# TARTRL/Deepfake_Detection

Measured on NVIDIA H100. Metric: images/sec (device-timed, max over ranks) efficientnet_b0 3x224x224 train step, higher is better.
Workload: dtype bf16

## Files before the change

### deepfake_detection_b200/csrc/dwconv.cu

```cuda
#include <stdlib.h>

#include "common.cuh"
#include "bn_finalize.cuh"

namespace {

constexpr int CB = 64;
constexpr int P = 8;
constexpr int NTHREADS = 256;
constexpr int DW_MAX_SMEM = 200 * 1024;


struct DwGeom {
    int N, H, W, C, Ho, Wo, pad;
    int TH, TW;
    int IH, IW;
    int tiles_x, tiles_y;
    int dbg;
    float* part;
};

__device__ __forceinline__ void load_chan_params(const float* p, int cbase, int C, float* out, float dflt) {
#pragma unroll
    for (int i = 0; i < 8; i++) out[i] = (p && cbase + i < C) ? p[cbase + i] : dflt;
}

constexpr int UNR = 4;
template <typename T, int ACT, bool AFFINE, int CPW = 32>
__device__ __forceinline__ void stage_input_tile(uint32_t* tile, const T* __restrict__ img, int H, int W, int C,
                                                 int c0, int iy0, int ix0, int IH, int IW,
                                                 const float* __restrict__ scale, const float* __restrict__ shift) {
    constexpr int VPP = CPW / 4;
    const int v = threadIdx.x % VPP;
    const int cbase = c0 + v * 8;
    const bool cvalid = cbase < C;
    float sc[8], sh[8];
    if (AFFINE) { load_chan_params(scale, cbase, C, sc, 1.f); load_chan_params(shift, cbase, C, sh, 0.f); }
    const int npix = IH * IW;
    const int PSTEP = blockDim.x / VPP;
    const int dq = PSTEP / IW, dr = PSTEP - dq * IW;
    int r = (threadIdx.x / VPP) / IW, c = (threadIdx.x / VPP) - r * IW;
    for (int base = threadIdx.x / VPP; base < npix; base += PSTEP * UNR) {
        uint4 raw[UNR];
        bool ok[UNR];
#pragma unroll
        for (int u = 0; u < UNR; u++) {
            const int pix = base + u * PSTEP;
// ... 15 lines not shown
#pragma unroll
                    for (int i = 0; i < 8; i++) {
                        float uu = AFFINE ? fmaf(f[i], sc[i], sh[i]) : f[i];
                        f[i] = act_fwd<ACT>(uu);
                    }
                    o = pack8<T>(f);
                } else {
                    o = raw[u];
                }
            }
            *reinterpret_cast<uint4*>(tile + pix * CPW + v * 4) = o;
        }
    }
}

template <typename T, bool AFFINE, int UG_ = 0, int CPW = 32>
__device__ __forceinline__ void stage_grad_tile(uint32_t* tile, const T* __restrict__ g, const T* __restrict__ y,
                                                int Ho, int Wo, int C, int c0, int oy0, int ox0, int IH, int IW,
                                                const float* __restrict__ cA, const float* __restrict__ cB,
                                                const float* __restrict__ cC) {
    constexpr int VPP = CPW / 4;
    const int v = threadIdx.x % VPP;
    const int cbase = c0 + v * 8;
    const bool cvalid = cbase < C;
    float A[8], B[8], Cc[8];
    if (AFFINE) { load_chan_params(cA, cbase, C, A, 1.f); load_chan_params(cB, cbase, C, B, 0.f); load_chan_params(cC, cbase, C, Cc, 0.f); }
    const int npix = IH * IW;
    const int PSTEP = blockDim.x / VPP;
    constexpr int UG = UG_ ? UG_ : (AFFINE ? 2 : 4);
    const int dq = PSTEP / IW, dr = PSTEP - dq * IW;
    int r = (threadIdx.x / VPP) / IW, c = (threadIdx.x / VPP) - r * IW;
    for (int base = threadIdx.x / VPP; base < npix; base += PSTEP * UG) {
        uint4 graw[UG], yraw[UG];
        bool ok[UG];
#pragma unroll
        for (int u = 0; u < UG; u++) {
            const int pix = base + u * PSTEP;
            const int oy = oy0 + r, ox = ox0 + c;
            ok[u] = pix < npix && cvalid && oy >= 0 && oy < Ho && ox >= 0 && ox < Wo;
            if (ok[u]) {
                const uint32_t off = (uint32_t)((oy * Wo + ox) * C + cbase);
                graw[u] = ldg16(g + off);
                if (AFFINE) yraw[u] = ldg16(y + off);
            }
// ... 10 lines not shown
                    float gg[8], yy[8];
                    unpack8<T>(graw[u], gg);
                    unpack8<T>(yraw[u], yy);
#pragma unroll
                    for (int i = 0; i < 8; i++) gg[i] = fmaf(A[i], gg[i], fmaf(B[i], yy[i], Cc[i]));
                    o = pack8<T>(gg);
                } else {
                    o = graw[u];
                }
            }
            *reinterpret_cast<uint4*>(tile + pix * CPW + v * 4) = o;
        }
    }
}

template <typename T, int K>
__device__ __forceinline__ void strip_dgrad_s2(const uint32_t* __restrict__ tile, int IW, int sy, int sx, int lane,
                                               const float (&w)[K * K][2], float (&acc)[P][2]) {
    constexpr int PAD = (K - 1) / 2;
#pragma unroll
    for (int kh = 0; kh < K; kh++) {
        const int q = sy + PAD - kh;
        if (q & 1) continue;
        const int row = (q >> 1) + 1;
        const uint32_t* rp = tile + (row * IW + (sx >> 1)) * 32 + lane;
        float2 vv[P / 2 + 2];
#pragma unroll
        for (int j = 0; j < P / 2 + 2; j++) vv[j] = unpack2<T>(rp[j * 32]);
#pragma unroll
        for (int p = 0; p < P; p++) {
// ... 45 lines not shown
    }
    __syncthreads();
    if (threadIdx.x < 2 * CPW) {
        float s = 0.f;
#pragma unroll
        for (int w = 0; w < (int)(blockDim.x >> 5); w++) s += sm[w * 64 + threadIdx.x];
        fn(threadIdx.x, s);
    }
    __syncthreads();
}

template <typename T, int K, int S, int ACT, bool AFFINE, int NT, int CPW = 32, int DT = 0, int DL = 0>
__global__ void __launch_bounds__(NT)
dwconv_fwd_kernel(const T* __restrict__ x, const float* __restrict__ scale, const float* __restrict__ shift,
                  const float* __restrict__ wgt, T* __restrict__ out, double* __restrict__ dsum,
                  double* __restrict__ dsq, const BnFinDesc* __restrict__ fin, DwGeom g) {
    extern __shared__ __align__(16) uint32_t tile[];
    __shared__ float red[NTHREADS / 32 * 64];
    constexpr int SUB = 32 / CPW;
    const int warp = threadIdx.x >> 5, lane = threadIdx.x & 31;
    const int cp = lane % CPW, sub = lane / CPW;
    const int tx = blockIdx.x % g.tiles_x, ty = blockIdx.x / g.tiles_x;
    const int c0 = blockIdx.y * (2 * CPW), n = blockIdx.z;
    const int oy0 = ty * g.TH, ox0 = tx * g.TW;
    const T* img = x + (size_t)n * g.H * g.W * g.C;
    stage_input_tile<T, ACT, AFFINE, CPW>(tile, img, g.H, g.W, g.C, c0, oy0 * S - (g.pad - DT), ox0 * S - (g.pad - DL), g.IH, g.IW, scale, shift);

    const int ch = c0 + cp * 2;
    const bool chv = ch < g.C;
    float w[K * K][2];
#pragma unroll
    for (int i = 0; i < K * K; i++) {
        w[i][0] = chv ? wgt[(size_t)ch * K * K + i] : 0.f;
        w[i][1] = chv ? wgt[(size_t)(ch + 1) * K * K + i] : 0.f;
    }
    __syncthreads();

    float s0 = 0.f, s1 = 0.f, q0 = 0.f, q1 = 0.f;
    const int strips_x = g.TW / P;
    const int xsh = 31 - __clz(strips_x);
    const int nstrips = ((g.TH + SUB - 1) / SUB) * strips_x;
    T* oimg = out + (size_t)n * g.Ho * g.Wo * g.C;
    for (int s = warp; s < nstrips; s += (int)(blockDim.x >> 5)) {
        const int sy = (s >> xsh) * SUB + sub, sx = (s & (strips_x - 1)) * P;
        int oy = oy0 + sy, ox = ox0 + sx;
        if (sy >= g.TH || oy >= g.Ho || ox >= g.Wo) continue;
        float acc[P][2];
#pragma unroll
        for (int p = 0; p < P; p++) { acc[p][0] = 0.f; acc[p][1] = 0.f; }
        strip_conv<T, K, S, CPW>(tile, g.IW, sy * S, sx * S, cp, w, acc);
        if (chv) {
#pragma unroll
            for (int p = 0; p < P; p++) {
                if (ox + p < g.Wo) {
                    uint32_t pk = pack2<T>(acc[p][0], acc[p][1]);
                    *reinterpret_cast<uint32_t*>(oimg + (uint32_t)((oy * g.Wo + ox + p) * g.C + ch)) = pk;
                    float2 r = unpack2<T>(pk);
                    s0 += r.x; s1 += r.y;
                    q0 = fmaf(r.x, r.x, q0); q1 = fmaf(r.y, r.y, q1);
                }
            }
        }
    }
    if (dsum) {
        double* ps = stat_slot(dsum, g.C);
        double* pq = stat_slot(dsq, g.C);
        reduce_warps_emit<CPW>(red, s0, s1, [&](int c, float v) { if (c0 + c < g.C) atomicAdd(ps + c0 + c, (double)v); });
        reduce_warps_emit<CPW>(red, q0, q1, [&](int c, float v) { if (c0 + c < g.C) atomicAdd(pq + c0 + c, (double)v); });
    }
    bn_finalize_tail(fin, threadIdx.x, NT);
}

template <typename T, int K, int S, int MODE, bool AFFINE, int NT>
__global__ void __launch_bounds__(NT)
dwconv_dgrad_kernel(const T* __restrict__ gy, const T* __restrict__ yout, const float* __restrict__ cA,
                    const float* __restrict__ cB, const float* __restrict__ cC, const float* __restrict__ wgt,
                    const T* __restrict__ xin, const float* __restrict__ scale, const float* __restrict__ shift,
                    const float* __restrict__ mean, const float* __restrict__ rstd, const T* __restrict__ add,
                    T* __restrict__ gx, double* __restrict__ ds1, double* __restrict__ ds2, DwGeom g) {
    extern __shared__ __align__(16) uint32_t tile[];
    __shared__ float red[NTHREADS / 32 * 64];
// ... 217 lines not shown
        }
    }
}

template <typename T, int K, int S, bool AFFINE, int MODE, int NT, int P, int CPW = 32, int DT = 0, int DL = 0>
#ifndef DW_BWD_OCC3
#define DW_BWD_OCC3 4
#endif
__global__ void __launch_bounds__(NT, K == 3 ? (P == 4 ? DW_BWD_OCC3 : 3) : 2)
dwconv_bwd_kernel(const T* __restrict__ gy, const T* __restrict__ yout, const float* __restrict__ cA,
                  const float* __restrict__ cB, const float* __restrict__ cC, const float* __restrict__ wgt,
                  const T* __restrict__ xin, const float* __restrict__ scale, const float* __restrict__ shift,
                  const float* __restrict__ mean, const float* __restrict__ rstd, const T* __restrict__ add,
                  T* __restrict__ gx,
                  float* __restrict__ dW, double* __restrict__ ds1, double* __restrict__ ds2,
                  const BnBwdFinDesc* __restrict__ fin, DwGeom g) {
    extern __shared__ __align__(16) uint32_t tile[];
    __shared__ float red[NTHREADS / 32 * 64];
    const int warp = threadIdx.x >> 5, lane = threadIdx.x & 31;
    constexpr int NW = NT / 32;
    constexpr int SUB = 32 / CPW;
    constexpr int CW = 2 * CPW;
    const int cp = lane % CPW, sub = lane / CPW;
    const int tx = blockIdx.x % g.tiles_x, ty = blockIdx.x / g.tiles_x;
    const int c0 = blockIdx.y * CW;
    const int y0 = ty * g.TH, x0 = tx * g.TW;
    const int pp = K - 1 - g.pad;
    const int ch = c0 + cp * 2;
    const bool chv = ch < g.C;
    float w[K * K][2], wacc[K * K][2];
#pragma unroll
    for (int i = 0; i < K * K; i++) {
        const int src = S == 1 ? (K * K - 1 - i) : i;
// ... 7 lines not shown
        mu0 = mean[ch]; mu1 = mean[ch + 1]; rs0 = rstd[ch]; rs1 = rstd[ch + 1];
    }
    const float nm0 = -mu0 * rs0, nm1 = -mu1 * rs1;
    float a0 = 0.f, a1 = 0.f, b0 = 0.f, b1 = 0.f;
    const int strips_x = g.TW / P;
    const int xsh = 31 - __clz(strips_x);
    const int row_groups = S == 1 ? (g.TH + SUB - 1) / SUB : ((g.TH + 1) / 2 + SUB - 1) / SUB;
    const int nstrips = (S == 1 ? row_groups : 2 * row_groups) * strips_x;
    auto strip_row = [&](int s) {
        const int r = s >> xsh;
        if (S == 1) return r * SUB + sub;
        const int par = r >= row_groups ? 1 : 0;
        return 2 * ((r - par * row_groups) * SUB + sub) + par;
    };

    for (int n = blockIdx.z; n < g.N; n += gridDim.z) {
        const size_t ooff = (size_t)n * g.Ho * g.Wo * g.C;
        const size_t ioff = (size_t)n * g.H * g.W * g.C;
        const T* xin_n = xin + ioff;
        T* gx_n = gx + ioff;
        uint32_t pre[P];
        auto prefetch = [&](int s) {
            const int sy = strip_row(s), sx = (s & (strips_x - 1)) * P;
            const int iy = y0 + sy, ix = x0 + sx;
            const bool rowok = chv && sy < g.TH && iy < g.H;
            const uint32_t off0 = (uint32_t)((iy * g.W + ix) * g.C + ch);
#pragma unroll
            for (int p = 0; p < P; p++)
                pre[p] = (rowok && ix + p < g.W) ? __ldg(reinterpret_cast<const uint32_t*>(xin_n + off0 + (uint32_t)(p * g.C))) : 0u;
        };
        if (warp < nstrips) prefetch(warp);
        __syncthreads();
        if (!(g.dbg & 2))
            stage_grad_tile<T, AFFINE, (K == 5 ? 4 : 2), CPW>(tile, gy + ooff, AFFINE ? yout + ooff : nullptr, g.Ho, g.Wo, g.C, c0,
                                   S == 1 ? y0 - pp : (y0 >> 1) - 1, S == 1 ? x0 - pp : (x0 >> 1) - 1, g.IH, g.IW, cA, cB, cC);
        __syncthreads();
        if (!(g.dbg & 1))
        for (int s = warp; s < nstrips; s += NW) {
            const int sy = strip_row(s), sx = (s & (strips_x - 1)) * P;
            const int iy = y0 + sy, ix = x0 + sx;
            float av[P][2], da[P][2], xh[P][2];
            const bool interior = sy < g.TH && iy < g.H && ix + P <= g.W;
#pragma unroll
            for (int p = 0; p < P; p++) {
                const float2 xi = unpack2<T>(pre[p]);
                if (MODE == 1) {
                    const float u0 = fmaf(xi.x, sc0, sh0), u1 = fmaf(xi.y, sc1, sh1);
                    const float g0 = sigmoid_fast(u0), g1 = sigmoid_fast(u1);
                    const float2 ar = unpack2<T>(pack2<T>(u0 * g0, u1 * g1));
                    av[p][0] = ar.x;
                    av[p][1] = ar.y;
// ... 193 lines not shown
    } while (0)

extern "C" {

static int dw_fwd(const void* x, const float* scale, const float* shift, const float* w, void* out, int N, int H, int W,
                  int C, int k, int stride, int dt_, int dl_, int act_in, int dt, double* dsum, double* dsq,
                  const void* fin, void* stream) {
    if (C % 8 || N <= 0 || H <= 0 || W <= 0) return dfd_set_error(DFD_ERR_ARG, "dfd_dwconv_fwd: sizes");
    const bool relu = act_in == DFD_ACT_RELU;
    if (relu && (k != 3 || stride != 1 || dt_ || dl_ || dsum || dsq || fin))
        return dfd_set_error(DFD_ERR_UNSUPPORTED, "dfd_dwconv_fwd: a ReLU input needs k = 3, stride 1 and no statistics");
    if (!relu && !scale && act_in != DFD_ACT_NONE) return dfd_set_error(DFD_ERR_ARG, "dfd_dwconv_fwd: act without BN");
    if (!relu && scale && act_in != DFD_ACT_SWISH) return dfd_set_error(DFD_ERR_UNSUPPORTED, "dfd_dwconv_fwd: BN input implies Swish");
    DwGeom g;
    const int cpw = dw_cpw(C);
    int smem = fill_geom(g, N, H, W, C, k, stride, false, cpw);
    if (dt_ || dl_) {
        if (stride != 2 || !scale || dw_nt(k) != (k == 5 ? 128 : 256))
            return dfd_set_error(DFD_ERR_UNSUPPORTED, "dfd_dwconv_fwd_pad: asymmetric pads need stride 2, a BN + Swish input and the default CTA size");
        dim3 grid(g.tiles_x * g.tiles_y, (C + 2 * cpw - 1) / (2 * cpw), N);
        cudaStream_t st = (cudaStream_t)stream;
#define FWP1(K_, CPW_, DT_, DL_) do { constexpr int NT = K_ == 5 ? 128 : 256;                                                  \
        DW_LAUNCH((dwconv_fwd_kernel<T, K_, 2, DFD_ACT_SWISH, true, NT, CPW_, DT_, DL_>), grid, smem, st, (const T*)x, scale, shift, w, \
                  (T*)out, dsum, dsq, (const BnFinDesc*)fin, g); } while (0)
#define FWP2(K_, DT_, DL_) do { if (cpw == 32) FWP1(K_, 32, DT_, DL_); else if (cpw == 16) FWP1(K_, 16, DT_, DL_); else FWP1(K_, 8, DT_, DL_); } while (0)
#define FWP(K_) do { if (dt_ && dl_) FWP2(K_, 1, 1); else if (dt_) FWP2(K_, 1, 0); else FWP2(K_, 0, 1); } while (0)
        DW_DISPATCH_T(dt, {
            if (k == 3) FWP(3);
            else if (k == 5) FWP(5);
            else return dfd_set_error(DFD_ERR_UNSUPPORTED, "depthwise conv: k in {3,5}, stride in {1,2}");
        });
#undef FWP
#undef FWP2
#undef FWP1
        DFD_LAUNCH_CHECK();
        return DFD_OK;
    }
    dim3 grid(g.tiles_x * g.tiles_y, (C + 2 * cpw - 1) / (2 * cpw), N);
    cudaStream_t st = (cudaStream_t)stream;
#define FW(ACT_, AFF_, CPW_) DW_LAUNCH((dwconv_fwd_kernel<T, K, S, ACT_, AFF_, NT, CPW_>), grid, smem, st, (const T*)x, scale, shift, w, (T*)out, dsum, dsq, (const BnFinDesc*)fin, g)
#define FWC(ACT_, AFF_) do { if (cpw == 32) FW(ACT_, AFF_, 32); else if (cpw == 16) FW(ACT_, AFF_, 16); else FW(ACT_, AFF_, 8); } while (0)
    if (relu) {
        DW_DISPATCH_T(dt, { constexpr int K = 3, S = 1; DW_NT(3, {
            if (scale) FWC(DFD_ACT_RELU, true);
            else FWC(DFD_ACT_RELU, false);
        }); });
        DFD_LAUNCH_CHECK();
        return DFD_OK;
    }
    DW_DISPATCH_T(dt, DW_DISPATCH_KS(k, stride, {
        if (scale) FWC(DFD_ACT_SWISH, true);
        else FWC(DFD_ACT_NONE, false);
    }));
#undef FWC
#undef FW
// ... 82 lines not shown
    return tiles * gz;
}

static int dw_bwd(const void* gy, const void* yout, const float* cA, const float* cB, const float* cC,
                  const float* w, const void* xin, const float* scale, const float* shift, const float* mean,
                  const float* rstd, const void* add, void* gx, float* dW, int N, int H, int W, int C, int k,
                  int stride, int dt_, int dl_, int dt, double* s1, double* s2, void* ws, long long ws_bytes, const void* fin,
                  void* stream, bool relu = false) {
    if (C % 8 || N <= 0 || H <= 0 || W <= 0) return dfd_set_error(DFD_ERR_ARG, "dfd_dwconv_bwd: sizes");
    if (relu && (k != 3 || stride != 1 || cA || dt_ || dl_))
        return dfd_set_error(DFD_ERR_UNSUPPORTED, "dfd_dwconv_bwd_relu: k = 3, stride 1, the BN backward not folded into gy (cA NULL)");
    if (!xin || !dW) return dfd_set_error(DFD_ERR_ARG, "dfd_dwconv_bwd: operands");
    if (scale && (!shift || !mean || !rstd || !s1 || !s2)) return dfd_set_error(DFD_ERR_ARG, "dfd_dwconv_bwd: mode 1 operands");
    DwGeom g;
    const int cpw = dw_cpw(C);
    int smem = fill_geom(g, N, H, W, C, k, stride, true, cpw);
    constexpr int NT = 128;
    const int red_bytes = (NT / 32) * k * k * 2 * cpw * (int)sizeof(float);
    if (smem < red_bytes) smem = red_bytes;
    int tiles, cbs, gz;
    dw_bwd_grid(g, N, C, cpw, tiles, cbs, gz);
    if (ws) {
        if ((long long)cbs * tiles * gz * k * k * 2 * cpw * 4 > ws_bytes)
            return dfd_set_error(DFD_ERR_ARG, "dfd_dwconv_bwd: workspace too small (blocks x dfd_dwconv_bwd_parts x block_channels*k*k floats)");
        g.part = (float*)ws;
    }
    dim3 grid(tiles, cbs, gz);
    cudaStream_t st = (cudaStream_t)stream;
    static int pb3 = 0, pb5 = 0;
    if (!pb3) { const char* e3 = getenv("DFD_DW_PB3"); const char* e5 = getenv("DFD_DW_PB5"); pb3 = (e3 && atoi(e3) == 8) ? 8 : 4; pb5 = (e5 && atoi(e5) == 4) ? 4 : 8; }
    const int pb = k == 3 ? pb3 : pb5;
#define BWARGS (const T*)gy, (const T*)yout, cA, cB, cC, w, (const T*)xin, scale, shift, mean, rstd, (const T*)add, (T*)gx, dW, s1, s2, (const BnBwdFinDesc*)fin, g
#define BW1(K_, S_, AFF, MODE_) do {                                                                                          \
        constexpr int PD = K_ == 3 ? 4 : 8;                                                                                   \
        if (cpw == 16) DW_LAUNCH((dwconv_bwd_kernel<T, K_, S_, AFF, MODE_, NT, PD, 16>), grid, smem, st, BWARGS);             \
        else if (cpw == 8) DW_LAUNCH((dwconv_bwd_kernel<T, K_, S_, AFF, MODE_, NT, PD, 8>), grid, smem, st, BWARGS);          \
        else if (pb == 4) DW_LAUNCH((dwconv_bwd_kernel<T, K_, S_, AFF, MODE_, NT, 4>), grid, smem, st, BWARGS);               \
        else DW_LAUNCH((dwconv_bwd_kernel<T, K_, S_, AFF, MODE_, NT, 8>), grid, smem, st, BWARGS);                            \
    } while (0)
#define BW(K_, S_) do { if (scale) { if (cA) BW1(K_, S_, true, 1); else BW1(K_, S_, false, 1); } else { if (cA) BW1(K_, S_, true, 0); else BW1(K_, S_, false, 0); } } while (0)
#define BWP1(K_, DT_, DL_) do {                                                                                               \
        constexpr int PD = K_ == 3 ? 4 : 8;                                                                                   \
        if (cpw == 16) DW_LAUNCH((dwconv_bwd_kernel<T, K_, 2, true, 1, NT, PD, 16, DT_, DL_>), grid, smem, st, BWARGS);       \
        else if (cpw == 8) DW_LAUNCH((dwconv_bwd_kernel<T, K_, 2, true, 1, NT, PD, 8, DT_, DL_>), grid, smem, st, BWARGS);    \
        else DW_LAUNCH((dwconv_bwd_kernel<T, K_, 2, true, 1, NT, PD, 32, DT_, DL_>), grid, smem, st, BWARGS);                 \
    } while (0)
#define BWP(K_) do { if (dt_ && dl_) BWP1(K_, 1, 1); else if (dt_) BWP1(K_, 1, 0); else BWP1(K_, 0, 1); } while (0)
// ... 62 lines not shown
```

### deepfake_detection_b200/csrc/gemm_tc.cu

```cuda
#include <cuda.h>
#include <stdio.h>
#include <stdlib.h>

#include <type_traits>

#include "common.cuh"
#include "bn_finalize.cuh"

namespace {

constexpr int BLOCK_M = 128;
constexpr int BLOCK_K = 64;
constexpr int MMA_K = 16;
constexpr int SLAB = 64;
constexpr int NUM_THREADS = 384;
constexpr int EPI_THREADS = 256;
constexpr int MAX_BLOCK_N = 128;
constexpr int SMEM_BUDGET = 224 * 1024;

__device__ __forceinline__ uint32_t smem_addr(const void* p) { return (uint32_t)__cvta_generic_to_shared(p); }

__device__ __forceinline__ void mbar_init(uint64_t* bar, uint32_t count) {
    asm volatile("mbarrier.init.shared::cta.b64 [%0], %1;" ::"r"(smem_addr(bar)), "r"(count));
}
__device__ __forceinline__ void mbar_arrive_expect_tx(uint64_t* bar, uint32_t bytes) {
    asm volatile("mbarrier.arrive.expect_tx.shared::cta.b64 _, [%0], %1;" ::"r"(smem_addr(bar)), "r"(bytes) : "memory");
}
__device__ __forceinline__ void mbar_arrive(uint64_t* bar) {
    asm volatile("mbarrier.arrive.shared::cta.b64 _, [%0];" ::"r"(smem_addr(bar)) : "memory");
}
__device__ __forceinline__ void mbar_wait(uint64_t* bar, uint32_t parity) {
    uint32_t addr = smem_addr(bar);
    asm volatile(
        "{\n"
        ".reg .pred p;\n"
        "WAIT_LOOP:\n"
        "mbarrier.try_wait.parity.shared::cta.b64 p, [%0], %1;\n"
        "@p bra WAIT_DONE;\n"
        "bra WAIT_LOOP;\n"
        "WAIT_DONE:\n"
        "}\n" ::"r"(addr), "r"(parity) : "memory");
}

__device__ __forceinline__ void tma_load_2d(void* smem_dst, const CUtensorMap* map, uint64_t* bar, int c0, int c1) {
    asm volatile(
        "cp.async.bulk.tensor.2d.shared::cluster.global.mbarrier::complete_tx::bytes [%0], [%1, {%3, %4}], [%2];"
        ::"r"(smem_addr(smem_dst)), "l"(reinterpret_cast<uint64_t>(map)), "r"(smem_addr(bar)), "r"(c0), "r"(c1)
        : "memory");
}
__device__ __forceinline__ void tma_store_2d(const CUtensorMap* map, const void* smem_src, int c0, int c1) {
    asm volatile("cp.async.bulk.tensor.2d.global.shared::cta.bulk_group [%0, {%2, %3}], [%1];"
                 ::"l"(reinterpret_cast<uint64_t>(map)), "r"(smem_addr(smem_src)), "r"(c0), "r"(c1) : "memory");
}
__device__ __forceinline__ void tma_load_4d(void* smem_dst, const CUtensorMap* map, uint64_t* bar, int c0, int c1, int c2, int c3) {
    asm volatile(
        "cp.async.bulk.tensor.4d.shared::cluster.global.mbarrier::complete_tx::bytes [%0], [%1, {%3, %4, %5, %6}], [%2];"
        ::"r"(smem_addr(smem_dst)), "l"(reinterpret_cast<uint64_t>(map)), "r"(smem_addr(bar)), "r"(c0), "r"(c1), "r"(c2), "r"(c3)
        : "memory");
}
__device__ __forceinline__ void tma_store_4d(const CUtensorMap* map, const void* smem_src, int c0, int c1, int c2, int c3) {
    asm volatile("cp.async.bulk.tensor.4d.global.shared::cta.bulk_group [%0, {%2, %3, %4, %5}], [%1];"
                 ::"l"(reinterpret_cast<uint64_t>(map)), "r"(smem_addr(smem_src)), "r"(c0), "r"(c1), "r"(c2), "r"(c3) : "memory");
}
__device__ __forceinline__ void tma_reduce_add_4d(const CUtensorMap* map, const void* smem_src, int c0, int c1, int c2, int c3) {
    asm volatile("cp.reduce.async.bulk.tensor.4d.global.shared::cta.add.tile.bulk_group [%0, {%2, %3, %4, %5}], [%1];"
                 ::"l"(reinterpret_cast<uint64_t>(map)), "r"(smem_addr(smem_src)), "r"(c0), "r"(c1), "r"(c2), "r"(c3) : "memory");
}
__device__ __forceinline__ void tma_store_commit() { asm volatile("cp.async.bulk.commit_group;" ::: "memory"); }
template <int N> __device__ __forceinline__ void tma_store_wait_read() {
    asm volatile("cp.async.bulk.wait_group.read %0;" ::"n"(N) : "memory");
}
__device__ __forceinline__ void prefetch_tmap(const CUtensorMap* map) {
    asm volatile("prefetch.tensormap [%0];" ::"l"(reinterpret_cast<uint64_t>(map)) : "memory");
}

__device__ __forceinline__ void wgmma_fence() { asm volatile("wgmma.fence.sync.aligned;" ::: "memory"); }
__device__ __forceinline__ void wgmma_commit() { asm volatile("wgmma.commit_group.sync.aligned;" ::: "memory"); }
template <int N> __device__ __forceinline__ void wgmma_wait() { asm volatile("wgmma.wait_group.sync.aligned %0;" ::"n"(N) : "memory"); }
__device__ __forceinline__ void wgmma_wait_all() { wgmma_wait<0>(); }
template <int R> __device__ __forceinline__ void fence_acc(float (&d)[R]) {
#pragma unroll
    for (int i = 0; i < R; i++) asm volatile("" : "+f"(d[i])::"memory");
}

template <typename T, int TA, int TB>
__device__ __forceinline__ void wgmma_n64(float (&d)[32], uint64_t adesc, uint64_t bdesc, uint32_t accumulate) {
    if constexpr (std::is_same<T, bf16>::value) {
        asm volatile(
            "{\n.reg .pred p;\nsetp.ne.b32 p, %34, 0;\n"
// ... 435 lines not shown
    for (int j = 0; j < BN / 8; j++) {
        const float s0 = odd ? acc[4 * j] : acc[4 * j + 2], s1 = odd ? acc[4 * j + 1] : acc[4 * j + 3];
        const float o0 = __shfl_xor_sync(0xffffffffu, s0, 1), o1 = __shfl_xor_sync(0xffffffffu, s1, 1);
        const float4 v = odd ? make_float4(o0, o1, acc[4 * j + 2], acc[4 * j + 3]) : make_float4(acc[4 * j], acc[4 * j + 1], o0, o1);
        const int col = n0 + 8 * j + cb;
        if (8 * j < p.block_n && row < p.Nw && col < p.Kw) {
            float* dst = base + (size_t)row * p.Kw + col;
            if (p.part) *reinterpret_cast<float4*>(dst) = v;
            else
                asm volatile("red.global.add.v4.f32 [%0], {%1, %2, %3, %4};" ::"l"(dst), "f"(v.x), "f"(v.y), "f"(v.z), "f"(v.w)
                             : "memory");
        }
    }
}

typedef CUresult (*EncodeTiledFn)(CUtensorMap*, CUtensorMapDataType, cuuint32_t, void*, const cuuint64_t*,
                                  const cuuint64_t*, const cuuint32_t*, const cuuint32_t*, CUtensorMapInterleave,
                                  CUtensorMapSwizzle, CUtensorMapL2promotion, CUtensorMapFloatOOBfill);

static EncodeTiledFn get_encode_fn() {
    static EncodeTiledFn fn = nullptr;
    if (!fn) {
        void* p = nullptr;
        cudaDriverEntryPointQueryResult qres;
        if (cudaGetDriverEntryPoint("cuTensorMapEncodeTiled", &p, cudaEnableDefault, &qres) == cudaSuccess &&
            qres == cudaDriverEntryPointSuccess)
            fn = (EncodeTiledFn)p;
    }
    return fn;
}

static int make_map(CUtensorMap* m, const void* base, long long rows, int cols, int box_rows, int is_bf16) {
    EncodeTiledFn fn = get_encode_fn();
    if (!fn) return dfd_set_error(DFD_ERR_CUDA, "cuTensorMapEncodeTiled entry point not available");
    cuuint64_t dims[2] = {(cuuint64_t)cols, (cuuint64_t)rows};
    cuuint64_t strides[1] = {(cuuint64_t)cols * 2};
    cuuint32_t box[2] = {(cuuint32_t)BLOCK_K, (cuuint32_t)box_rows};
    cuuint32_t estr[2] = {1, 1};
    CUresult r = fn(m, is_bf16 ? CU_TENSOR_MAP_DATA_TYPE_BFLOAT16 : CU_TENSOR_MAP_DATA_TYPE_FLOAT16, 2,
                    const_cast<void*>(base), dims, strides, box, estr, CU_TENSOR_MAP_INTERLEAVE_NONE,
                    CU_TENSOR_MAP_SWIZZLE_128B, CU_TENSOR_MAP_L2_PROMOTION_L2_256B, CU_TENSOR_MAP_FLOAT_OOB_FILL_NONE);
    if (r != CUDA_SUCCESS) {
        char buf[160];
        snprintf(buf, sizeof(buf), "cuTensorMapEncodeTiled failed (%d) rows=%lld cols=%d box_rows=%d", (int)r, rows, cols, box_rows);
        return dfd_set_error(DFD_ERR_CUDA, buf);
    }
    return DFD_OK;
}


struct PixelView { long long sW, sH, sN; };
static int make_map_nhwc(CUtensorMap* m, const void* base, int N, int H, int W, int C, int bw, int bh, int bn, int is_bf16,
                         int es = 1, const PixelView* pv = nullptr) {
    EncodeTiledFn fn = get_encode_fn();
    if (!fn) return dfd_set_error(DFD_ERR_CUDA, "cuTensorMapEncodeTiled entry point not available");
    cuuint64_t dims[4] = {(cuuint64_t)C, (cuuint64_t)W, (cuuint64_t)H, (cuuint64_t)N};
    cuuint64_t strides[3] = {(cuuint64_t)C * 2, (cuuint64_t)W * C * 2, (cuuint64_t)H * W * C * 2};
    if (pv) { strides[0] = (cuuint64_t)pv->sW; strides[1] = (cuuint64_t)pv->sH; strides[2] = (cuuint64_t)pv->sN; }
    cuuint32_t box[4] = {(cuuint32_t)BLOCK_K, (cuuint32_t)((bw - 1) * es + 1), (cuuint32_t)((bh - 1) * es + 1), (cuuint32_t)bn};
    cuuint32_t estr[4] = {1, (cuuint32_t)es, (cuuint32_t)es, 1};
    CUresult r = fn(m, is_bf16 ? CU_TENSOR_MAP_DATA_TYPE_BFLOAT16 : CU_TENSOR_MAP_DATA_TYPE_FLOAT16, 4,
                    const_cast<void*>(base), dims, strides, box, estr, CU_TENSOR_MAP_INTERLEAVE_NONE,
                    CU_TENSOR_MAP_SWIZZLE_128B, CU_TENSOR_MAP_L2_PROMOTION_L2_256B, CU_TENSOR_MAP_FLOAT_OOB_FILL_NONE);
    if (r != CUDA_SUCCESS) {
        char buf[200];
        snprintf(buf, sizeof(buf), "cuTensorMapEncodeTiled (4-D) failed (%d) N=%d H=%d W=%d C=%d box=%dx%dx%d", (int)r, N, H, W, C, bw, bh, bn);
        return dfd_set_error(DFD_ERR_CUDA, buf);
    }
    return DFD_OK;
}

template <typename T, int BN>
static void launch_tc_kernel(int grid, size_t smem, cudaStream_t st, const CUtensorMap& ma, const CUtensorMap& mb,
                             const CUtensorMap& mc, const TcParams& p) {
    static bool attr = false;
    if (!attr) { cudaFuncSetAttribute(gemm_tc_kernel<T, BN>, cudaFuncAttributeMaxDynamicSharedMemorySize, SMEM_BUDGET); attr = true; }
    gemm_tc_kernel<T, BN><<<grid, NUM_THREADS, smem, st>>>(ma, mb, mc, p);
}

template <typename T, int BN>
static void launch_wgrad_kernel(dim3 grid, size_t smem, cudaStream_t st, const CUtensorMap& mg, const CUtensorMap& mx, float* dW,
                                const WgParams& p) {
    static bool attr = false;
    if (!attr) { cudaFuncSetAttribute(wgrad_tc_kernel<T, BN>, cudaFuncAttributeMaxDynamicSharedMemorySize, 100 * 1024); attr = true; }
    wgrad_tc_kernel<T, BN><<<grid, WG_THREADS, smem, st>>>(mg, mx, dW, p);
// ... 315 lines not shown
```

Before: 11470.

## Stage depthwise conv input and gradient tiles via TMA with double-buffered prefetch

```diff
diff --git a/deepfake_detection_b200/csrc/dwconv.cu b/deepfake_detection_b200/csrc/dwconv.cu
--- a/deepfake_detection_b200/csrc/dwconv.cu
+++ b/deepfake_detection_b200/csrc/dwconv.cu
@@ -2,6 +2,7 @@
 
 #include "common.cuh"
 #include "bn_finalize.cuh"
+#include "tma.cuh"
 
 namespace {
 
@@ -26,11 +27,11 @@
 }
 
 constexpr int UNR = 4;
-template <typename T, int ACT, bool AFFINE, int CPW = 32>
+template <typename T, int ACT, bool AFFINE>
 __device__ __forceinline__ void stage_input_tile(uint32_t* tile, const T* __restrict__ img, int H, int W, int C,
                                                  int c0, int iy0, int ix0, int IH, int IW,
                                                  const float* __restrict__ scale, const float* __restrict__ shift) {
-    constexpr int VPP = CPW / 4;
+    constexpr int CPW = 32, VPP = CPW / 4;
     const int v = threadIdx.x % VPP;
     const int cbase = c0 + v * 8;
     const bool cvalid = cbase < C;
@@ -76,12 +77,12 @@
     }
 }
 
-template <typename T, bool AFFINE, int UG_ = 0, int CPW = 32>
+template <typename T, bool AFFINE>
 __device__ __forceinline__ void stage_grad_tile(uint32_t* tile, const T* __restrict__ g, const T* __restrict__ y,
                                                 int Ho, int Wo, int C, int c0, int oy0, int ox0, int IH, int IW,
                                                 const float* __restrict__ cA, const float* __restrict__ cB,
                                                 const float* __restrict__ cC) {
-    constexpr int VPP = CPW / 4;
+    constexpr int CPW = 32, VPP = CPW / 4;
     const int v = threadIdx.x % VPP;
     const int cbase = c0 + v * 8;
     const bool cvalid = cbase < C;
@@ -89,7 +90,7 @@
     if (AFFINE) { load_chan_params(cA, cbase, C, A, 1.f); load_chan_params(cB, cbase, C, B, 0.f); load_chan_params(cC, cbase, C, Cc, 0.f); }
     const int npix = IH * IW;
     const int PSTEP = blockDim.x / VPP;
-    constexpr int UG = UG_ ? UG_ : (AFFINE ? 2 : 4);
+    constexpr int UG = AFFINE ? 2 : 4;
     const int dq = PSTEP / IW, dr = PSTEP - dq * IW;
     int r = (threadIdx.x / VPP) / IW, c = (threadIdx.x / VPP) - r * IW;
     for (int base = threadIdx.x / VPP; base < npix; base += PSTEP * UG) {
@@ -130,6 +131,76 @@
     }
 }
 
+template <typename T, int ACT, bool AFFINE, int CPW>
+__device__ __forceinline__ void activate_tile(uint32_t* __restrict__ tile, int H, int W, int C, int c0, int iy0, int ix0,
+                                              int IH, int IW, const float* __restrict__ scale, const float* __restrict__ shift) {
+    constexpr int VPP = CPW / 4;
+    const int v = threadIdx.x % VPP;
+    const int cbase = c0 + v * 8;
+    const bool cvalid = cbase < C;
+    float sc[8], sh[8];
+    if (AFFINE) { load_chan_params(scale, cbase, C, sc, 1.f); load_chan_params(shift, cbase, C, sh, 0.f); }
+    const int npix = IH * IW;
+    const int PSTEP = blockDim.x / VPP;
+    const int dq = PSTEP / IW, dr = PSTEP - dq * IW;
+    int r = (threadIdx.x / VPP) / IW, c = (threadIdx.x / VPP) - r * IW;
+#pragma unroll 4
+    for (int pix = threadIdx.x / VPP; pix < npix; pix += PSTEP) {
+        const int iy = iy0 + r, ix = ix0 + c;
+        const bool ok = cvalid && iy >= 0 && iy < H && ix >= 0 && ix < W;
+        uint4* q = reinterpret_cast<uint4*>(tile + pix * CPW + v * 4);
+        uint4 o = make_uint4(0, 0, 0, 0);
+        if (ok) {
+            float f[8];
+            unpack8<T>(*q, f);
+#pragma unroll
+            for (int i = 0; i < 8; i++) f[i] = act_fwd<ACT>(AFFINE ? fmaf(f[i], sc[i], sh[i]) : f[i]);
+            o = pack8<T>(f);
+        }
+        *q = o;
+        r += dq; c += dr;
+        if (c >= IW) { c -= IW; r++; }
+    }
+}
+
+template <typename T, bool AFFINE, int CPW>
+__device__ __forceinline__ void form_grad_tile(uint32_t* __restrict__ dyt, const uint32_t* __restrict__ rg,
+                                               const uint32_t* __restrict__ ry, int Ho, int Wo, int C, int c0, int oy0,
+                                               int ox0, int IH, int IW, const float* __restrict__ cA,
+                                               const float* __restrict__ cB, const float* __restrict__ cC) {
+    constexpr int VPP = CPW / 4;
+    const int v = threadIdx.x % VPP;
+    const int cbase = c0 + v * 8;
+    const bool cvalid = cbase < C;
+    float A[8], B[8], Cc[8];
+    if (AFFINE) { load_chan_params(cA, cbase, C, A, 1.f); load_chan_params(cB, cbase, C, B, 0.f); load_chan_params(cC, cbase, C, Cc, 0.f); }
+    const int npix = IH * IW;
+    const int PSTEP = blockDim.x / VPP;
+    const int dq = PSTEP / IW, dr = PSTEP - dq * IW;
+    int r = (threadIdx.x / VPP) / IW, c = (threadIdx.x / VPP) - r * IW;
+#pragma unroll 4
+    for (int pix = threadIdx.x / VPP; pix < npix; pix += PSTEP) {
+        const int oy = oy0 + r, ox = ox0 + c;
+        const bool ok = cvalid && oy >= 0 && oy < Ho && ox >= 0 && ox < Wo;
+        const int off = pix * CPW + v * 4;
+        uint4 o = make_uint4(0, 0, 0, 0);
+        if (ok) {
+            o = *reinterpret_cast<const uint4*>(rg + off);
+            if (AFFINE) {
+                float gg[8], yy[8];
+                unpack8<T>(o, gg);
+                unpack8<T>(*reinterpret_cast<const uint4*>(ry + off), yy);
+#pragma unroll
+                for (int i = 0; i < 8; i++) gg[i] = fmaf(A[i], gg[i], fmaf(B[i], yy[i], Cc[i]));
+                o = pack8<T>(gg);
+            }
+        }
+        *reinterpret_cast<uint4*>(dyt + off) = o;
+        r += dq; c += dr;
+        if (c >= IW) { c -= IW; r++; }
+    }
+}
+
 template <typename T, int K>
 __device__ __forceinline__ void strip_dgrad_s2(const uint32_t* __restrict__ tile, int IW, int sy, int sx, int lane,
                                                const float (&w)[K * K][2], float (&acc)[P][2]) {
@@ -205,17 +276,25 @@
 __global__ void __launch_bounds__(NT)
 dwconv_fwd_kernel(const T* __restrict__ x, const float* __restrict__ scale, const float* __restrict__ shift,
                   const float* __restrict__ wgt, T* __restrict__ out, double* __restrict__ dsum,
-                  double* __restrict__ dsq, const BnFinDesc* __restrict__ fin, DwGeom g) {
-    extern __shared__ __align__(16) uint32_t tile[];
-    __shared__ float red[NTHREADS / 32 * 64];
+                  double* __restrict__ dsq, const BnFinDesc* __restrict__ fin, DwGeom g,
+                  const __grid_constant__ CUtensorMap tm_x) {
+    extern __shared__ __align__(16) uint32_t smem_dyn[];
+    __shared__ uint64_t full;
+    const uint32_t sa = smem_addr(smem_dyn);
+    uint32_t* const tile = smem_dyn + ((((sa + 127u) & ~127u) - sa) >> 2);
     constexpr int SUB = 32 / CPW;
     const int warp = threadIdx.x >> 5, lane = threadIdx.x & 31;
     const int cp = lane % CPW, sub = lane / CPW;
     const int tx = blockIdx.x % g.tiles_x, ty = blockIdx.x / g.tiles_x;
     const int c0 = blockIdx.y * (2 * CPW), n = blockIdx.z;
     const int oy0 = ty * g.TH, ox0 = tx * g.TW;
-    const T* img = x + (size_t)n * g.H * g.W * g.C;
-    stage_input_tile<T, ACT, AFFINE, CPW>(tile, img, g.H, g.W, g.C, c0, oy0 * S - (g.pad - DT), ox0 * S - (g.pad - DL), g.IH, g.IW, scale, shift);
+    const int iy0 = oy0 * S - (g.pad - DT), ix0 = ox0 * S - (g.pad - DL);
+    if (threadIdx.x == 0) {
+        mbar_init(&full, 1);
+        asm volatile("fence.mbarrier_init.release.cluster;" ::: "memory");
+        mbar_arrive_expect_tx(&full, (uint32_t)(g.IH * g.IW * CPW * 4));
+        tma_load_4d(tile, &tm_x, &full, c0, ix0, iy0, n);
+    }
 
     const int ch = c0 + cp * 2;
     const bool chv = ch < g.C;
@@ -226,6 +305,11 @@
         w[i][1] = chv ? wgt[(size_t)(ch + 1) * K * K + i] : 0.f;
     }
     __syncthreads();
+    mbar_wait(&full, 0);
+    if (AFFINE || ACT != DFD_ACT_NONE) {
+        activate_tile<T, ACT, AFFINE, CPW>(tile, g.H, g.W, g.C, c0, iy0, ix0, g.IH, g.IW, scale, shift);
+        __syncthreads();
+    }
 
     float s0 = 0.f, s1 = 0.f, q0 = 0.f, q1 = 0.f;
     const int strips_x = g.TW / P;
@@ -256,6 +340,8 @@
     if (dsum) {
         double* ps = stat_slot(dsum, g.C);
         double* pq = stat_slot(dsq, g.C);
+        float* red = reinterpret_cast<float*>(tile);
+        __syncthreads();
         reduce_warps_emit<CPW>(red, s0, s1, [&](int c, float v) { if (c0 + c < g.C) atomicAdd(ps + c0 + c, (double)v); });
         reduce_warps_emit<CPW>(red, q0, q1, [&](int c, float v) { if (c0 + c < g.C) atomicAdd(pq + c0 + c, (double)v); });
     }
@@ -503,9 +589,11 @@
                   const float* __restrict__ mean, const float* __restrict__ rstd, const T* __restrict__ add,
                   T* __restrict__ gx,
                   float* __restrict__ dW, double* __restrict__ ds1, double* __restrict__ ds2,
-                  const BnBwdFinDesc* __restrict__ fin, DwGeom g) {
+                  const BnBwdFinDesc* __restrict__ fin, DwGeom g,
+                  const __grid_constant__ CUtensorMap tm_gy, const __grid_constant__ CUtensorMap tm_yout) {
     extern __shared__ __align__(16) uint32_t tile[];
     __shared__ float red[NTHREADS / 32 * 64];
+    __shared__ uint64_t full;
     const int warp = threadIdx.x >> 5, lane = threadIdx.x & 31;
     constexpr int NW = NT / 32;
     constexpr int SUB = 32 / CPW;
@@ -543,8 +631,24 @@
         return 2 * ((r - par * row_groups) * SUB + sub) + par;
     };
 
+    const int oy0 = S == 1 ? y0 - pp : (y0 >> 1) - 1, ox0 = S == 1 ? x0 - pp : (x0 >> 1) - 1;
+    const int tile_words = (g.IH * g.IW * CPW + 31) & ~31;
+    const uint32_t tile_sa = smem_addr(tile);
+    uint32_t* const rg = tile + ((((tile_sa + (uint32_t)tile_words * 4u + 127u) & ~127u) - tile_sa) >> 2);
+    uint32_t* const ry = rg + tile_words;
+    auto fetch = [&](int n) {
+        mbar_arrive_expect_tx(&full, (AFFINE ? 2u : 1u) * (uint32_t)(g.IH * g.IW * CPW * 4));
+        tma_load_4d(rg, &tm_gy, &full, c0, ox0, oy0, n);
+        if (AFFINE) tma_load_4d(ry, &tm_yout, &full, c0, ox0, oy0, n);
+    };
+    if (threadIdx.x == 0) {
+        mbar_init(&full, 1);
+        asm volatile("fence.mbarrier_init.release.cluster;" ::: "memory");
+        fetch(blockIdx.z);
+    }
+    uint32_t phase = 0;
+
     for (int n = blockIdx.z; n < g.N; n += gridDim.z) {
-        const size_t ooff = (size_t)n * g.Ho * g.Wo * g.C;
         const size_t ioff = (size_t)n * g.H * g.W * g.C;
         const T* xin_n = xin + ioff;
         T* gx_n = gx + ioff;
@@ -560,10 +664,14 @@
         };
         if (warp < nstrips) prefetch(warp);
         __syncthreads();
-        if (!(g.dbg & 2))
-            stage_grad_tile<T, AFFINE, (K == 5 ? 4 : 2), CPW>(tile, gy + ooff, AFFINE ? yout + ooff : nullptr, g.Ho, g.Wo, g.C, c0,
-                                   S == 1 ? y0 - pp : (y0 >> 1) - 1, S == 1 ? x0 - pp : (x0 >> 1) - 1, g.IH, g.IW, cA, cB, cC);
+        mbar_wait(&full, phase);
+        phase ^= 1;
+        form_grad_tile<T, AFFINE, CPW>(tile, rg, ry, g.Ho, g.Wo, g.C, c0, oy0, ox0, g.IH, g.IW, cA, cB, cC);
         __syncthreads();
+        if (threadIdx.x == 0 && n + (int)gridDim.z < g.N) {
+            asm volatile("fence.proxy.async.shared::cta;" ::: "memory");
+            fetch(n + gridDim.z);
+        }
         if (!(g.dbg & 1))
         for (int s = warp; s < nstrips; s += NW) {
             const int sy = strip_row(s), sx = (s & (strips_x - 1)) * P;
@@ -787,7 +895,11 @@
     if (!relu && scale && act_in != DFD_ACT_SWISH) return dfd_set_error(DFD_ERR_UNSUPPORTED, "dfd_dwconv_fwd: BN input implies Swish");
     DwGeom g;
     const int cpw = dw_cpw(C);
-    int smem = fill_geom(g, N, H, W, C, k, stride, false, cpw);
+    const int tile_bytes = fill_geom(g, N, H, W, C, k, stride, false, cpw);
+    const int smem = (tile_bytes > NTHREADS / 32 * 64 * 4 ? tile_bytes : NTHREADS / 32 * 64 * 4) + 128;
+    CUtensorMap tm_x;
+    if (int rc = make_map_nhwc(&tm_x, x, N, H, W, C, g.IW, g.IH, 1, dt == DFD_DT_BF16, 1, nullptr, 2 * cpw,
+                               CU_TENSOR_MAP_SWIZZLE_NONE)) return rc;
     if (dt_ || dl_) {
         if (stride != 2 || !scale || dw_nt(k) != (k == 5 ? 128 : 256))
             return dfd_set_error(DFD_ERR_UNSUPPORTED, "dfd_dwconv_fwd_pad: asymmetric pads need stride 2, a BN + Swish input and the default CTA size");
@@ -795,7 +907,7 @@
         cudaStream_t st = (cudaStream_t)stream;
 #define FWP1(K_, CPW_, DT_, DL_) do { constexpr int NT = K_ == 5 ? 128 : 256;                                                  \
         DW_LAUNCH((dwconv_fwd_kernel<T, K_, 2, DFD_ACT_SWISH, true, NT, CPW_, DT_, DL_>), grid, smem, st, (const T*)x, scale, shift, w, \
-                  (T*)out, dsum, dsq, (const BnFinDesc*)fin, g); } while (0)
+                  (T*)out, dsum, dsq, (const BnFinDesc*)fin, g, tm_x); } while (0)
 #define FWP2(K_, DT_, DL_) do { if (cpw == 32) FWP1(K_, 32, DT_, DL_); else if (cpw == 16) FWP1(K_, 16, DT_, DL_); else FWP1(K_, 8, DT_, DL_); } while (0)
 #define FWP(K_) do { if (dt_ && dl_) FWP2(K_, 1, 1); else if (dt_) FWP2(K_, 1, 0); else FWP2(K_, 0, 1); } while (0)
         DW_DISPATCH_T(dt, {
@@ -811,7 +923,7 @@
     }
     dim3 grid(g.tiles_x * g.tiles_y, (C + 2 * cpw - 1) / (2 * cpw), N);
     cudaStream_t st = (cudaStream_t)stream;
-#define FW(ACT_, AFF_, CPW_) DW_LAUNCH((dwconv_fwd_kernel<T, K, S, ACT_, AFF_, NT, CPW_>), grid, smem, st, (const T*)x, scale, shift, w, (T*)out, dsum, dsq, (const BnFinDesc*)fin, g)
+#define FW(ACT_, AFF_, CPW_) DW_LAUNCH((dwconv_fwd_kernel<T, K, S, ACT_, AFF_, NT, CPW_>), grid, smem, st, (const T*)x, scale, shift, w, (T*)out, dsum, dsq, (const BnFinDesc*)fin, g, tm_x)
 #define FWC(ACT_, AFF_) do { if (cpw == 32) FW(ACT_, AFF_, 32); else if (cpw == 16) FW(ACT_, AFF_, 16); else FW(ACT_, AFF_, 8); } while (0)
     if (relu) {
         DW_DISPATCH_T(dt, { constexpr int K = 3, S = 1; DW_NT(3, {
@@ -924,10 +1036,19 @@
     if (scale && (!shift || !mean || !rstd || !s1 || !s2)) return dfd_set_error(DFD_ERR_ARG, "dfd_dwconv_bwd: mode 1 operands");
     DwGeom g;
     const int cpw = dw_cpw(C);
-    int smem = fill_geom(g, N, H, W, C, k, stride, true, cpw);
+    const int tile_bytes = fill_geom(g, N, H, W, C, k, stride, true, cpw);
+    int smem = (cA ? 3 : 2) * ((tile_bytes + 127) & ~127) + 128;
     constexpr int NT = 128;
     const int red_bytes = (NT / 32) * k * k * 2 * cpw * (int)sizeof(float);
     if (smem < red_bytes) smem = red_bytes;
+    CUtensorMap tm_gy, tm_yout;
+    if (int rc = make_map_nhwc(&tm_gy, gy, N, g.Ho, g.Wo, C, g.IW, g.IH, 1, dt == DFD_DT_BF16, 1, nullptr, 2 * cpw,
+                               CU_TENSOR_MAP_SWIZZLE_NONE)) return rc;
+    tm_yout = tm_gy;
+    if (cA) {
+        if (int rc = make_map_nhwc(&tm_yout, yout, N, g.Ho, g.Wo, C, g.IW, g.IH, 1, dt == DFD_DT_BF16, 1, nullptr, 2 * cpw,
+                                   CU_TENSOR_MAP_SWIZZLE_NONE)) return rc;
+    }
     int tiles, cbs, gz;
     dw_bwd_grid(g, N, C, cpw, tiles, cbs, gz);
     if (ws) {
@@ -940,7 +1061,7 @@
     static int pb3 = 0, pb5 = 0;
     if (!pb3) { const char* e3 = getenv("DFD_DW_PB3"); const char* e5 = getenv("DFD_DW_PB5"); pb3 = (e3 && atoi(e3) == 8) ? 8 : 4; pb5 = (e5 && atoi(e5) == 4) ? 4 : 8; }
     const int pb = k == 3 ? pb3 : pb5;
-#define BWARGS (const T*)gy, (const T*)yout, cA, cB, cC, w, (const T*)xin, scale, shift, mean, rstd, (const T*)add, (T*)gx, dW, s1, s2, (const BnBwdFinDesc*)fin, g
+#define BWARGS (const T*)gy, (const T*)yout, cA, cB, cC, w, (const T*)xin, scale, shift, mean, rstd, (const T*)add, (T*)gx, dW, s1, s2, (const BnBwdFinDesc*)fin, g, tm_gy, tm_yout
 #define BW1(K_, S_, AFF, MODE_) do {                                                                                          \
         constexpr int PD = K_ == 3 ? 4 : 8;                                                                                   \
         if (cpw == 16) DW_LAUNCH((dwconv_bwd_kernel<T, K_, S_, AFF, MODE_, NT, PD, 16>), grid, smem, st, BWARGS);             \
diff --git a/deepfake_detection_b200/csrc/gemm_tc.cu b/deepfake_detection_b200/csrc/gemm_tc.cu
--- a/deepfake_detection_b200/csrc/gemm_tc.cu
+++ b/deepfake_detection_b200/csrc/gemm_tc.cu
@@ -6,6 +6,7 @@
 
 #include "common.cuh"
 #include "bn_finalize.cuh"
+#include "tma.cuh"
 
 namespace {
 
@@ -17,62 +18,6 @@
 constexpr int EPI_THREADS = 256;
 constexpr int MAX_BLOCK_N = 128;
 constexpr int SMEM_BUDGET = 224 * 1024;
-
-__device__ __forceinline__ uint32_t smem_addr(const void* p) { return (uint32_t)__cvta_generic_to_shared(p); }
-
-__device__ __forceinline__ void mbar_init(uint64_t* bar, uint32_t count) {
-    asm volatile("mbarrier.init.shared::cta.b64 [%0], %1;" ::"r"(smem_addr(bar)), "r"(count));
-}
-__device__ __forceinline__ void mbar_arrive_expect_tx(uint64_t* bar, uint32_t bytes) {
-    asm volatile("mbarrier.arrive.expect_tx.shared::cta.b64 _, [%0], %1;" ::"r"(smem_addr(bar)), "r"(bytes) : "memory");
-}
-__device__ __forceinline__ void mbar_arrive(uint64_t* bar) {
-    asm volatile("mbarrier.arrive.shared::cta.b64 _, [%0];" ::"r"(smem_addr(bar)) : "memory");
-}
-__device__ __forceinline__ void mbar_wait(uint64_t* bar, uint32_t parity) {
-    uint32_t addr = smem_addr(bar);
-    asm volatile(
-        "{\n"
-        ".reg .pred p;\n"
-        "WAIT_LOOP:\n"
-        "mbarrier.try_wait.parity.shared::cta.b64 p, [%0], %1;\n"
-        "@p bra WAIT_DONE;\n"
-        "bra WAIT_LOOP;\n"
-        "WAIT_DONE:\n"
-        "}\n" ::"r"(addr), "r"(parity) : "memory");
-}
-
-__device__ __forceinline__ void tma_load_2d(void* smem_dst, const CUtensorMap* map, uint64_t* bar, int c0, int c1) {
-    asm volatile(
-        "cp.async.bulk.tensor.2d.shared::cluster.global.mbarrier::complete_tx::bytes [%0], [%1, {%3, %4}], [%2];"
-        ::"r"(smem_addr(smem_dst)), "l"(reinterpret_cast<uint64_t>(map)), "r"(smem_addr(bar)), "r"(c0), "r"(c1)
-        : "memory");
-}
-__device__ __forceinline__ void tma_store_2d(const CUtensorMap* map, const void* smem_src, int c0, int c1) {
-    asm volatile("cp.async.bulk.tensor.2d.global.shared::cta.bulk_group [%0, {%2, %3}], [%1];"
-                 ::"l"(reinterpret_cast<uint64_t>(map)), "r"(smem_addr(smem_src)), "r"(c0), "r"(c1) : "memory");
-}
-__device__ __forceinline__ void tma_load_4d(void* smem_dst, const CUtensorMap* map, uint64_t* bar, int c0, int c1, int c2, int c3) {
-    asm volatile(
-        "cp.async.bulk.tensor.4d.shared::cluster.global.mbarrier::complete_tx::bytes [%0], [%1, {%3, %4, %5, %6}], [%2];"
-        ::"r"(smem_addr(smem_dst)), "l"(reinterpret_cast<uint64_t>(map)), "r"(smem_addr(bar)), "r"(c0), "r"(c1), "r"(c2), "r"(c3)
-        : "memory");
-}
-__device__ __forceinline__ void tma_store_4d(const CUtensorMap* map, const void* smem_src, int c0, int c1, int c2, int c3) {
-    asm volatile("cp.async.bulk.tensor.4d.global.shared::cta.bulk_group [%0, {%2, %3, %4, %5}], [%1];"
-                 ::"l"(reinterpret_cast<uint64_t>(map)), "r"(smem_addr(smem_src)), "r"(c0), "r"(c1), "r"(c2), "r"(c3) : "memory");
-}
-__device__ __forceinline__ void tma_reduce_add_4d(const CUtensorMap* map, const void* smem_src, int c0, int c1, int c2, int c3) {
-    asm volatile("cp.reduce.async.bulk.tensor.4d.global.shared::cta.add.tile.bulk_group [%0, {%2, %3, %4, %5}], [%1];"
-                 ::"l"(reinterpret_cast<uint64_t>(map)), "r"(smem_addr(smem_src)), "r"(c0), "r"(c1), "r"(c2), "r"(c3) : "memory");
-}
-__device__ __forceinline__ void tma_store_commit() { asm volatile("cp.async.bulk.commit_group;" ::: "memory"); }
-template <int N> __device__ __forceinline__ void tma_store_wait_read() {
-    asm volatile("cp.async.bulk.wait_group.read %0;" ::"n"(N) : "memory");
-}
-__device__ __forceinline__ void prefetch_tmap(const CUtensorMap* map) {
-    asm volatile("prefetch.tensormap [%0];" ::"l"(reinterpret_cast<uint64_t>(map)) : "memory");
-}
 
 __device__ __forceinline__ void wgmma_fence() { asm volatile("wgmma.fence.sync.aligned;" ::: "memory"); }
 __device__ __forceinline__ void wgmma_commit() { asm volatile("wgmma.commit_group.sync.aligned;" ::: "memory"); }
@@ -538,21 +483,6 @@
     }
 }
 
-typedef CUresult (*EncodeTiledFn)(CUtensorMap*, CUtensorMapDataType, cuuint32_t, void*, const cuuint64_t*,
-                                  const cuuint64_t*, const cuuint32_t*, const cuuint32_t*, CUtensorMapInterleave,
-                                  CUtensorMapSwizzle, CUtensorMapL2promotion, CUtensorMapFloatOOBfill);
-
-static EncodeTiledFn get_encode_fn() {
-    static EncodeTiledFn fn = nullptr;
-    if (!fn) {
-        void* p = nullptr;
-        cudaDriverEntryPointQueryResult qres;
-        if (cudaGetDriverEntryPoint("cuTensorMapEncodeTiled", &p, cudaEnableDefault, &qres) == cudaSuccess &&
-            qres == cudaDriverEntryPointSuccess)
-            fn = (EncodeTiledFn)p;
-    }
-    return fn;
-}
 
 static int make_map(CUtensorMap* m, const void* base, long long rows, int cols, int box_rows, int is_bf16) {
     EncodeTiledFn fn = get_encode_fn();
@@ -572,27 +502,6 @@
     return DFD_OK;
 }
 
-
-struct PixelView { long long sW, sH, sN; };
-static int make_map_nhwc(CUtensorMap* m, const void* base, int N, int H, int W, int C, int bw, int bh, int bn, int is_bf16,
-                         int es = 1, const PixelView* pv = nullptr) {
-    EncodeTiledFn fn = get_encode_fn();
-    if (!fn) return dfd_set_error(DFD_ERR_CUDA, "cuTensorMapEncodeTiled entry point not available");
-    cuuint64_t dims[4] = {(cuuint64_t)C, (cuuint64_t)W, (cuuint64_t)H, (cuuint64_t)N};
-    cuuint64_t strides[3] = {(cuuint64_t)C * 2, (cuuint64_t)W * C * 2, (cuuint64_t)H * W * C * 2};
-    if (pv) { strides[0] = (cuuint64_t)pv->sW; strides[1] = (cuuint64_t)pv->sH; strides[2] = (cuuint64_t)pv->sN; }
-    cuuint32_t box[4] = {(cuuint32_t)BLOCK_K, (cuuint32_t)((bw - 1) * es + 1), (cuuint32_t)((bh - 1) * es + 1), (cuuint32_t)bn};
-    cuuint32_t estr[4] = {1, (cuuint32_t)es, (cuuint32_t)es, 1};
-    CUresult r = fn(m, is_bf16 ? CU_TENSOR_MAP_DATA_TYPE_BFLOAT16 : CU_TENSOR_MAP_DATA_TYPE_FLOAT16, 4,
-                    const_cast<void*>(base), dims, strides, box, estr, CU_TENSOR_MAP_INTERLEAVE_NONE,
-                    CU_TENSOR_MAP_SWIZZLE_128B, CU_TENSOR_MAP_L2_PROMOTION_L2_256B, CU_TENSOR_MAP_FLOAT_OOB_FILL_NONE);
-    if (r != CUDA_SUCCESS) {
-        char buf[200];
-        snprintf(buf, sizeof(buf), "cuTensorMapEncodeTiled (4-D) failed (%d) N=%d H=%d W=%d C=%d box=%dx%dx%d", (int)r, N, H, W, C, bw, bh, bn);
-        return dfd_set_error(DFD_ERR_CUDA, buf);
-    }
-    return DFD_OK;
-}
 
 template <typename T, int BN>
 static void launch_tc_kernel(int grid, size_t smem, cudaStream_t st, const CUtensorMap& ma, const CUtensorMap& mb,
diff --git a/deepfake_detection_b200/csrc/tma.cuh b/deepfake_detection_b200/csrc/tma.cuh
--- /dev/null
+++ b/deepfake_detection_b200/csrc/tma.cuh
@@ -0,0 +1,103 @@
+#pragma once
+#include <cuda.h>
+#include <stdio.h>
+
+#include "common.cuh"
+
+namespace {
+
+__device__ __forceinline__ uint32_t smem_addr(const void* p) { return (uint32_t)__cvta_generic_to_shared(p); }
+
+__device__ __forceinline__ void mbar_init(uint64_t* bar, uint32_t count) {
+    asm volatile("mbarrier.init.shared::cta.b64 [%0], %1;" ::"r"(smem_addr(bar)), "r"(count));
+}
+__device__ __forceinline__ void mbar_arrive_expect_tx(uint64_t* bar, uint32_t bytes) {
+    asm volatile("mbarrier.arrive.expect_tx.shared::cta.b64 _, [%0], %1;" ::"r"(smem_addr(bar)), "r"(bytes) : "memory");
+}
+__device__ __forceinline__ void mbar_arrive(uint64_t* bar) {
+    asm volatile("mbarrier.arrive.shared::cta.b64 _, [%0];" ::"r"(smem_addr(bar)) : "memory");
+}
+__device__ __forceinline__ void mbar_wait(uint64_t* bar, uint32_t parity) {
+    uint32_t addr = smem_addr(bar);
+    asm volatile(
+        "{\n"
+        ".reg .pred p;\n"
+        "WAIT_LOOP:\n"
+        "mbarrier.try_wait.parity.shared::cta.b64 p, [%0], %1;\n"
+        "@p bra WAIT_DONE;\n"
+        "bra WAIT_LOOP;\n"
+        "WAIT_DONE:\n"
+        "}\n" ::"r"(addr), "r"(parity) : "memory");
+}
+
+__device__ __forceinline__ void tma_load_2d(void* smem_dst, const CUtensorMap* map, uint64_t* bar, int c0, int c1) {
+    asm volatile(
+        "cp.async.bulk.tensor.2d.shared::cluster.global.mbarrier::complete_tx::bytes [%0], [%1, {%3, %4}], [%2];"
+        ::"r"(smem_addr(smem_dst)), "l"(reinterpret_cast<uint64_t>(map)), "r"(smem_addr(bar)), "r"(c0), "r"(c1)
+        : "memory");
+}
+__device__ __forceinline__ void tma_store_2d(const CUtensorMap* map, const void* smem_src, int c0, int c1) {
+    asm volatile("cp.async.bulk.tensor.2d.global.shared::cta.bulk_group [%0, {%2, %3}], [%1];"
+                 ::"l"(reinterpret_cast<uint64_t>(map)), "r"(smem_addr(smem_src)), "r"(c0), "r"(c1) : "memory");
+}
+__device__ __forceinline__ void tma_load_4d(void* smem_dst, const CUtensorMap* map, uint64_t* bar, int c0, int c1, int c2, int c3) {
+    asm volatile(
+        "cp.async.bulk.tensor.4d.shared::cluster.global.mbarrier::complete_tx::bytes [%0], [%1, {%3, %4, %5, %6}], [%2];"
+        ::"r"(smem_addr(smem_dst)), "l"(reinterpret_cast<uint64_t>(map)), "r"(smem_addr(bar)), "r"(c0), "r"(c1), "r"(c2), "r"(c3)
+        : "memory");
+}
+__device__ __forceinline__ void tma_store_4d(const CUtensorMap* map, const void* smem_src, int c0, int c1, int c2, int c3) {
+    asm volatile("cp.async.bulk.tensor.4d.global.shared::cta.bulk_group [%0, {%2, %3, %4, %5}], [%1];"
+                 ::"l"(reinterpret_cast<uint64_t>(map)), "r"(smem_addr(smem_src)), "r"(c0), "r"(c1), "r"(c2), "r"(c3) : "memory");
+}
+__device__ __forceinline__ void tma_reduce_add_4d(const CUtensorMap* map, const void* smem_src, int c0, int c1, int c2, int c3) {
+    asm volatile("cp.reduce.async.bulk.tensor.4d.global.shared::cta.add.tile.bulk_group [%0, {%2, %3, %4, %5}], [%1];"
+                 ::"l"(reinterpret_cast<uint64_t>(map)), "r"(smem_addr(smem_src)), "r"(c0), "r"(c1), "r"(c2), "r"(c3) : "memory");
+}
+__device__ __forceinline__ void tma_store_commit() { asm volatile("cp.async.bulk.commit_group;" ::: "memory"); }
+template <int N> __device__ __forceinline__ void tma_store_wait_read() {
+    asm volatile("cp.async.bulk.wait_group.read %0;" ::"n"(N) : "memory");
+}
+__device__ __forceinline__ void prefetch_tmap(const CUtensorMap* map) {
+    asm volatile("prefetch.tensormap [%0];" ::"l"(reinterpret_cast<uint64_t>(map)) : "memory");
+}
+
+typedef CUresult (*EncodeTiledFn)(CUtensorMap*, CUtensorMapDataType, cuuint32_t, void*, const cuuint64_t*,
+                                  const cuuint64_t*, const cuuint32_t*, const cuuint32_t*, CUtensorMapInterleave,
+                                  CUtensorMapSwizzle, CUtensorMapL2promotion, CUtensorMapFloatOOBfill);
+
+static EncodeTiledFn get_encode_fn() {
+    static EncodeTiledFn fn = nullptr;
+    if (!fn) {
+        void* p = nullptr;
+        cudaDriverEntryPointQueryResult qres;
+        if (cudaGetDriverEntryPoint("cuTensorMapEncodeTiled", &p, cudaEnableDefault, &qres) == cudaSuccess &&
+            qres == cudaDriverEntryPointSuccess)
+            fn = (EncodeTiledFn)p;
+    }
+    return fn;
+}
+
+struct PixelView { long long sW, sH, sN; };
+static int make_map_nhwc(CUtensorMap* m, const void* base, int N, int H, int W, int C, int bw, int bh, int bn, int is_bf16,
+                         int es = 1, const PixelView* pv = nullptr, int bc = 64,
+                         CUtensorMapSwizzle swz = CU_TENSOR_MAP_SWIZZLE_128B) {
+    EncodeTiledFn fn = get_encode_fn();
+    if (!fn) return dfd_set_error(DFD_ERR_CUDA, "cuTensorMapEncodeTiled entry point not available");
+    cuuint64_t dims[4] = {(cuuint64_t)C, (cuuint64_t)W, (cuuint64_t)H, (cuuint64_t)N};
+    cuuint64_t strides[3] = {(cuuint64_t)C * 2, (cuuint64_t)W * C * 2, (cuuint64_t)H * W * C * 2};
+    if (pv) { strides[0] = (cuuint64_t)pv->sW; strides[1] = (cuuint64_t)pv->sH; strides[2] = (cuuint64_t)pv->sN; }
+    cuuint32_t box[4] = {(cuuint32_t)bc, (cuuint32_t)((bw - 1) * es + 1), (cuuint32_t)((bh - 1) * es + 1), (cuuint32_t)bn};
+    cuuint32_t estr[4] = {1, (cuuint32_t)es, (cuuint32_t)es, 1};
+    CUresult r = fn(m, is_bf16 ? CU_TENSOR_MAP_DATA_TYPE_BFLOAT16 : CU_TENSOR_MAP_DATA_TYPE_FLOAT16, 4,
+                    const_cast<void*>(base), dims, strides, box, estr, CU_TENSOR_MAP_INTERLEAVE_NONE,
+                    swz, CU_TENSOR_MAP_L2_PROMOTION_L2_256B, CU_TENSOR_MAP_FLOAT_OOB_FILL_NONE);
+    if (r != CUDA_SUCCESS) {
+        char buf[200];
+        snprintf(buf, sizeof(buf), "cuTensorMapEncodeTiled (4-D) failed (%d) N=%d H=%d W=%d C=%d box=%dx%dx%d", (int)r, N, H, W, C, bw, bh, bn);
+        return dfd_set_error(DFD_ERR_CUDA, buf);
+    }
+    return DFD_OK;
+}
+
+}
```

Result: faster. 11850, median of 6 (+3.4%).
